# JunkyByte/easy_ViTPose

Measured on NVIDIA H100. Metric: person-crops/sec ViT-B 256x192 bf16, higher is better.
Workload: dtype bf16

## Files before the change

### easy_vitpose_b200/_lib.py

```python
from __future__ import annotations

import ctypes as C
import os

from .build import LIB, build, is_stale

_lib = None


class VpbConfig(C.Structure):
    _fields_ = [("embed_dim", C.c_int32), ("depth", C.c_int32), ("num_heads", C.c_int32),
                ("num_keypoints", C.c_int32), ("max_batch", C.c_int32), ("device", C.c_int32)]


MAX_FRAMES = 64


class VpbFrame(C.Structure):
    _fields_ = [("data", C.c_void_p), ("height", C.c_int32), ("width", C.c_int32), ("pitch_bytes", C.c_int64),
                ("num_boxes", C.c_int32), ("rotation", C.c_int32)]


ROTATIONS = (0, 90, 180, 270)
YUV_MATRICES = {"bt601": 0, "bt709": 1}
# ... 72 lines not shown
    "vpb_infer_frames": (C.c_int, [C.c_void_p, C.POINTER(VpbFrame), C.c_int32, C.c_void_p, C.c_void_p, C.c_void_p, C.c_void_p]),
    "vpb_infer_frames_host": (C.c_int, [C.c_void_p, C.POINTER(VpbFrame), C.c_int32, C.c_void_p, C.c_void_p, C.c_void_p, C.c_void_p]),
    "vpb_submit_frames_host": (C.c_int, [C.c_void_p, C.POINTER(VpbFrame), C.c_int32, C.c_void_p, C.c_void_p, C.c_void_p, C.c_int32]),
    "vpb_preprocess_affine": (C.c_int, [C.POINTER(VpbFrame), C.c_int32, C.c_void_p, C.c_void_p, C.c_void_p]),
    "vpb_infer_affine": (C.c_int, [C.c_void_p, C.POINTER(VpbFrame), C.c_int32, C.c_void_p, C.c_void_p, C.c_void_p, C.c_void_p,
                                   C.c_void_p]),
    "vpb_infer_affine_host": (C.c_int, [C.c_void_p, C.POINTER(VpbFrame), C.c_int32, C.c_void_p, C.c_void_p, C.c_void_p,
                                        C.c_void_p, C.c_void_p]),
    "vpb_create_heads": (C.c_int, [C.POINTER(VpbConfig), C.c_int32, C.c_void_p, C.c_int32, C.POINTER(C.c_void_p)]),
    "vpb_infer_heads": (C.c_int, [C.c_void_p, C.c_void_p, C.c_void_p, C.POINTER(VpbSegment), C.c_int32, C.c_void_p, C.c_void_p,
                                  C.c_void_p, C.c_void_p]),
    "vpb_infer_frames_heads": (C.c_int, [C.c_void_p, C.POINTER(VpbFrame), C.c_int32, C.c_void_p, C.c_void_p, C.c_void_p, C.c_void_p,
                                         C.c_void_p]),
    "vpb_infer_frames_heads_host": (C.c_int, [C.c_void_p, C.POINTER(VpbFrame), C.c_int32, C.c_void_p, C.c_void_p, C.c_void_p,
                                              C.c_void_p, C.c_void_p]),
    "vpb_infer_affine_heads": (C.c_int, [C.c_void_p, C.POINTER(VpbFrame), C.c_int32, C.c_void_p, C.c_void_p, C.c_void_p, C.c_void_p,
                                         C.c_void_p, C.c_void_p]),
    "vpb_infer_affine_heads_host": (C.c_int, [C.c_void_p, C.POINTER(VpbFrame), C.c_int32, C.c_void_p, C.c_void_p, C.c_void_p,
                                              C.c_void_p, C.c_void_p, C.c_void_p]),
    "vpb_infer_frames_yuv": (C.c_int, [C.c_void_p, C.POINTER(VpbFrameYuv), C.c_int32, C.c_int32, C.c_int32, C.c_int32, C.c_void_p,
                                       C.c_void_p, C.c_void_p, C.c_void_p]),
    "vpb_infer_frames_yuv_host": (C.c_int, [C.c_void_p, C.POINTER(VpbFrameYuv), C.c_int32, C.c_int32, C.c_int32, C.c_int32, C.c_void_p,
                                            C.c_void_p, C.c_void_p, C.c_void_p]),
    "vpb_submit_frames_yuv_host": (C.c_int, [C.c_void_p, C.POINTER(VpbFrameYuv), C.c_int32, C.c_int32, C.c_int32, C.c_int32, C.c_void_p,
                                             C.c_void_p, C.c_void_p, C.c_int32]),
    "vpb_infer_affine_yuv": (C.c_int, [C.c_void_p, C.POINTER(VpbFrameYuv), C.c_int32, C.c_int32, C.c_int32, C.c_int32, C.c_void_p,
                                       C.c_void_p, C.c_void_p, C.c_void_p, C.c_void_p]),
    "vpb_infer_affine_yuv_host": (C.c_int, [C.c_void_p, C.POINTER(VpbFrameYuv), C.c_int32, C.c_int32, C.c_int32, C.c_int32, C.c_void_p,
                                            C.c_void_p, C.c_void_p, C.c_void_p, C.c_void_p]),
    "vpb_infer_frames_heads_yuv": (C.c_int, [C.c_void_p, C.POINTER(VpbFrameYuv), C.c_int32, C.c_int32, C.c_int32, C.c_int32, C.c_void_p,
                                             C.c_void_p, C.c_void_p, C.c_void_p, C.c_void_p]),
    "vpb_infer_frames_heads_yuv_host": (C.c_int, [C.c_void_p, C.POINTER(VpbFrameYuv), C.c_int32, C.c_int32, C.c_int32, C.c_int32,
                                                  C.c_void_p, C.c_void_p, C.c_void_p, C.c_void_p, C.c_void_p]),
    "vpb_infer_affine_heads_yuv": (C.c_int, [C.c_void_p, C.POINTER(VpbFrameYuv), C.c_int32, C.c_int32, C.c_int32, C.c_int32, C.c_void_p,
                                             C.c_void_p, C.c_void_p, C.c_void_p, C.c_void_p, C.c_void_p]),
    "vpb_infer_affine_heads_yuv_host": (C.c_int, [C.c_void_p, C.POINTER(VpbFrameYuv), C.c_int32, C.c_int32, C.c_int32, C.c_int32,
                                                  C.c_void_p, C.c_void_p, C.c_void_p, C.c_void_p, C.c_void_p, C.c_void_p]),
    "vpb_host_alloc": (C.c_void_p, [C.c_int64]),
    "vpb_host_free": (None, [C.c_void_p]),
    "vpb_kernel_launches": (C.c_int, [C.c_void_p, C.c_int32]),
    "vpb_cached_graphs": (C.c_int, [C.c_void_p, C.c_int32, C.POINTER(C.c_int32), C.POINTER(C.c_int32)]),
    "vpb_device_bytes": (C.c_int64, [C.c_void_p]),
    "vpb_set_option": (C.c_int, [C.c_void_p, C.c_char_p, C.c_int32]),
    "vpb_set_flip_test": (C.c_int, [C.c_void_p, C.c_void_p, C.c_int32, C.c_int32]),
    "vpb_set_flip_test_heads": (C.c_int, [C.c_void_p, C.c_void_p, C.c_int32, C.c_int32]),
    "vpb_profile_classes": (C.c_int, []),
    "vpb_profile_class_name": (C.c_char_p, [C.c_int32]),
    "vpb_profile_collect": (C.c_int, [C.c_void_p, C.c_void_p, C.c_void_p]),
    "vpb_read_buffer": (C.c_int, [C.c_void_p, C.c_char_p, C.c_void_p, C.c_int64]),
    "vpb_gemm": (C.c_int, [C.c_void_p, C.c_void_p, C.c_void_p, C.c_void_p, C.c_int32, C.c_int32, C.c_int32, C.c_int32,
                           C.c_void_p, C.c_int32, C.c_int32, C.c_int32, C.c_int32, C.c_int32, C.c_void_p]),
    "vpb_debug_gemm": (C.c_int, [C.c_int32, C.c_void_p]),
    "vpb_attention": (C.c_int, [C.c_void_p, C.c_int32, C.c_int32, C.c_int32, C.c_void_p, C.c_void_p]),
    "vpb_debug_attention": (C.c_int, [C.c_int32]),
    "vpb_layernorm": (C.c_int, [C.c_void_p, C.c_void_p, C.c_void_p, C.c_void_p, C.c_int32, C.c_int32, C.c_float, C.c_void_p]),
    "vpb_draw_workspace_bytes": (C.c_int64, [C.c_int32, C.c_int32, C.c_int32]),
    "vpb_draw_poses": (C.c_int, [C.POINTER(VpbCanvas), C.c_int32, C.c_int32, C.c_void_p, C.c_int32, C.c_void_p, C.c_void_p, C.c_int32,
                                 C.c_void_p, C.c_int32, C.c_void_p, C.c_int32, C.c_int32, C.c_float, C.c_void_p, C.c_void_p]),
    "vpb_tracker_create": (C.c_int, [C.c_int32, C.c_int32, C.c_int32, C.c_double, C.c_int32, C.POINTER(C.c_void_p)]),
    "vpb_tracker_destroy": (None, [C.c_void_p]),
    "vpb_tracker_update": (C.c_int, [C.c_void_p, C.c_void_p, C.c_void_p, C.c_void_p, C.c_void_p, C.c_void_p, C.c_void_p]),
    "vpb_tracker_reset": (C.c_int, [C.c_void_p, C.c_int32, C.c_void_p]),
    "vpb_tracker_next_id": (C.c_int, [C.c_void_p, C.POINTER(C.c_int64)]),
    "vpb_tracker_set_next_id": (C.c_int, [C.c_void_p, C.c_int64]),
    "vpb_tracker_status": (C.c_int, [C.c_void_p, C.POINTER(C.c_int32)]),
    "vpb_smoother_create": (C.c_int, [C.c_int32, C.c_int32, C.c_double, C.c_double, C.c_double, C.c_double, C.c_double, C.c_int32,
                                      C.c_int32, C.POINTER(C.c_void_p)]),
    "vpb_smoother_destroy": (None, [C.c_void_p]),
    "vpb_smoother_update": (C.c_int, [C.c_void_p, C.c_void_p, C.c_int32, C.c_void_p, C.c_void_p, C.c_void_p, C.c_void_p, C.c_void_p]),
    "vpb_smoother_reset": (C.c_int, [C.c_void_p, C.c_int32, C.c_void_p]),
    "vpb_smoother_status": (C.c_int, [C.c_void_p, C.POINTER(C.c_int32)]),
    "vpb_oks_nms": (C.c_int, [C.c_void_p, C.c_int32, C.c_int32, C.c_void_p, C.c_int32, C.c_void_p, C.c_void_p, C.c_void_p,
                              C.POINTER(VpbOksNmsParams), C.c_void_p, C.c_void_p, C.c_void_p, C.c_void_p, C.c_void_p]),
    "vpb_oks_iou": (C.c_int, [C.c_void_p, C.c_int32, C.c_int32, C.c_void_p, C.c_int32, C.c_void_p, C.c_void_p, C.c_double,
                              C.c_void_p, C.c_void_p, C.c_void_p]),
    "vpb_coco_eval_workspace_bytes": (C.c_int64, [C.c_int32, C.c_int32]),
    "vpb_coco_eval": (C.c_int, [C.c_int32, C.c_void_p, C.POINTER(VpbCocoGts), C.POINTER(VpbCocoDets), C.c_void_p, C.c_int64, C.c_void_p,
                                C.c_void_p, C.c_void_p, C.c_void_p, C.c_void_p]),
}

EXPORTS_NV12 = {
    "vpb_infer_frames_nv12": (C.c_int, [C.c_void_p, C.POINTER(VpbFrameNv12), C.c_int32, C.c_int32, C.c_void_p, C.c_void_p, C.c_void_p,
                                        C.c_void_p]),
    "vpb_infer_frames_nv12_host": (C.c_int, [C.c_void_p, C.POINTER(VpbFrameNv12), C.c_int32, C.c_int32, C.c_void_p, C.c_void_p,
                                             C.c_void_p, C.c_void_p]),
    "vpb_submit_frames_nv12_host": (C.c_int, [C.c_void_p, C.POINTER(VpbFrameNv12), C.c_int32, C.c_int32, C.c_void_p, C.c_void_p,
                                              C.c_void_p, C.c_int32]),
    "vpb_infer_affine_nv12": (C.c_int, [C.c_void_p, C.POINTER(VpbFrameNv12), C.c_int32, C.c_int32, C.c_void_p, C.c_void_p, C.c_void_p,
                                        C.c_void_p, C.c_void_p]),
    "vpb_infer_affine_nv12_host": (C.c_int, [C.c_void_p, C.POINTER(VpbFrameNv12), C.c_int32, C.c_int32, C.c_void_p, C.c_void_p,
                                             C.c_void_p, C.c_void_p, C.c_void_p]),
}


def lib():
    global _lib
    if _lib is None:
        if not os.path.exists(LIB) or is_stale():
            try:
                build()
            except Exception as exc:
                if not os.path.exists(LIB) or os.environ.get("VPB_ALLOW_STALE", "0") != "1":
                    raise RuntimeError(f"{LIB} is missing or older than its sources and could not be rebuilt ({exc}); build it "
                                       "with `python -m easy_vitpose_b200.build`; there is no fallback implementation") from exc
                import warnings
                warnings.warn(f"loading a STALE {LIB} (VPB_ALLOW_STALE=1): {exc}")
# ... 19 lines not shown
```

### easy_vitpose_b200/csrc/attention.cuh

```cuda
#pragma once
#include <cuda.h>

#include "ptx.cuh"
#include "wgmma.cuh"

namespace vpb {

constexpr int ATT_T = 192;
constexpr int ATT_THREADS = 3 * 128;

template <int HD>
struct AttCfg {
  static_assert(HD == 32 || HD == 64 || HD == 80, "head_dim");
  static constexpr int MAIN = HD == 32 ? 32 : 64;
  static constexpr int TAIL = HD - MAIN;
  static constexpr int MAIN_ROW = MAIN * 2;
  static constexpr int MAIN_BYTES = ATT_T * MAIN_ROW;
  static constexpr int TAIL_BYTES = TAIL ? ATT_T * 32 : 0;
  static constexpr int OPER_BYTES = MAIN_BYTES + TAIL_BYTES;
  static constexpr int STAGE_BYTES = 3 * OPER_BYTES;
  static constexpr int SMEM = 2 * STAGE_BYTES + 1024  + 256 ;
  static_assert(OPER_BYTES % 1024 == 0 && MAIN_BYTES % 1024 == 0, "swizzled boxes keep 1024-byte alignment");
};

struct AttnParams {
  int batch;
  int heads;
  int dim;
  __nv_bfloat16* out;
  long long* dbg;
};

template <int HD, int NPOLY, typename OperandsDone>
__device__ __forceinline__ void attend_item(uint32_t sQ, uint32_t sK, uint32_t sV, __nv_bfloat16* out, int dim, int b, int head, int wg,
                                            int lane, int wq, OperandsDone&& operands_done) {
  using Cfg = AttCfg<HD>;
  static_assert(NPOLY == 0 || NPOLY == 8, "NPOLY");
  constexpr float kLog2e = 1.4426950408889634f;
  float s[ATT_T / 2];
  wgmma_fence();
  {
    const uint64_t qd = wgmma_desc<Cfg::MAIN_ROW>(sQ + wg * 64 * Cfg::MAIN_ROW), kd = wgmma_desc<Cfg::MAIN_ROW>(sK);
#pragma unroll
    for (int k = 0; k < Cfg::MAIN / 16; ++k) wgmma_ss<ATT_T>(s, qd + 2 * k, kd + 2 * k, k != 0);
    if constexpr (Cfg::TAIL > 0)
      wgmma_ss<ATT_T>(s, wgmma_desc<32>(sQ + Cfg::MAIN_BYTES + wg * 64 * 32), wgmma_desc<32>(sK + Cfg::MAIN_BYTES), 1);
  }
  wgmma_commit();
  wgmma_wait<0>();
  wgmma_fence_regs(s);

  float sum[2];
#pragma unroll
  for (int h = 0; h < 2; ++h) {
    float mx = -INFINITY;
#pragma unroll
    for (int j = 0; j < ATT_T / 8; ++j) mx = fmaxf(mx, fmaxf(s[4 * j + 2 * h], s[4 * j + 2 * h + 1]));
    mx = fmaxf(mx, __shfl_xor_sync(0xffffffffu, mx, 1));
    mx = fmaxf(mx, __shfl_xor_sync(0xffffffffu, mx, 2));
    const float mscaled = mx * kLog2e;
    float sm = 0.0f;
#pragma unroll
    for (int j = 0; j < ATT_T / 8; ++j) {
      const float a1 = fmaf(s[4 * j + 2 * h + 1], kLog2e, -mscaled);
      const float e0 = __bfloat162float(__float2bfloat16_rn(ex2_approx(fmaf(s[4 * j + 2 * h], kLog2e, -mscaled))));
      const float e1 = __bfloat162float(__float2bfloat16_rn((NPOLY > 0 && (j & 1) == 0) ? ex2_poly(a1) : ex2_approx(a1)));
      sm += e0 + e1;
      s[4 * j + 2 * h] = e0;
      s[4 * j + 2 * h + 1] = e1;
    }
    sm += __shfl_xor_sync(0xffffffffu, sm, 1);
    sm += __shfl_xor_sync(0xffffffffu, sm, 2);
    sum[h] = sm;
  }

  float o[Cfg::MAIN / 2];
  [[maybe_unused]] float ot[8];
  wgmma_fence();
#pragma unroll
  for (int kk = 0; kk < ATT_T / 16; ++kk) {
    uint32_t a[4];
    a[0] = pack_bf16(s[8 * kk + 0], s[8 * kk + 1]);
    a[1] = pack_bf16(s[8 * kk + 2], s[8 * kk + 3]);
    a[2] = pack_bf16(s[8 * kk + 4], s[8 * kk + 5]);
    a[3] = pack_bf16(s[8 * kk + 6], s[8 * kk + 7]);
    const uint64_t vd = wgmma_desc<Cfg::MAIN_ROW>(sV + kk * 16 * Cfg::MAIN_ROW);
    if constexpr (Cfg::MAIN == 64) wgmma_rs_n64<1>(o, a, vd, kk != 0);
    else wgmma_rs_n32<1>(o, a, vd, kk != 0);
    if constexpr (Cfg::TAIL > 0) wgmma_rs_n16<1>(ot, a, wgmma_desc<32>(sV + Cfg::MAIN_BYTES + kk * 16 * 32), kk != 0);
  }
  wgmma_commit();
  wgmma_wait<0>();
  wgmma_fence_regs(o);
  if constexpr (Cfg::TAIL > 0) wgmma_fence_regs(ot);

  operands_done();

  const int r_lo = wg * 64 + wq * 16 + (lane >> 2);
  const int cq = 2 * (lane & 3);
#pragma unroll
  for (int hh = 0; hh < 2; ++hh) {
    const float inv = 1.0f / sum[hh];
    __nv_bfloat16* orow = out + (static_cast<size_t>(b) * ATT_T + r_lo + 8 * hh) * dim + head * HD;
#pragma unroll
    for (int j = 0; j < Cfg::MAIN / 8; ++j)
      *reinterpret_cast<uint32_t*>(orow + 8 * j + cq) = pack_bf16(o[4 * j + 2 * hh] * inv, o[4 * j + 2 * hh + 1] * inv);
    if constexpr (Cfg::TAIL > 0) {
#pragma unroll
      for (int j = 0; j < 2; ++j)
        *reinterpret_cast<uint32_t*>(orow + Cfg::MAIN + 8 * j + cq) = pack_bf16(ot[4 * j + 2 * hh] * inv, ot[4 * j + 2 * hh + 1] * inv);
    }
  }
}

template <int HD, int NPOLY = 0>
__global__ void __launch_bounds__(ATT_THREADS, 1)
attention_wgmma(const __grid_constant__ CUtensorMap tmap_main, const __grid_constant__ CUtensorMap tmap_tail, const AttnParams p) {
  using Cfg = AttCfg<HD>;
  extern __shared__ uint8_t smem_raw[];
  uint8_t* smem = reinterpret_cast<uint8_t*>((reinterpret_cast<uintptr_t>(smem_raw) + 1023) & ~uintptr_t(1023));
  uint64_t* full = reinterpret_cast<uint64_t*>(smem + 2 * Cfg::STAGE_BYTES);

  const int wg = threadIdx.x >> 7;
  const int tid = threadIdx.x & 127;
  const int lane = threadIdx.x & 31, wq = tid >> 5;
  const int items = p.batch * p.heads;
  const long long t_cta0 = p.dbg ? clock64() : 0;
  long long t_wait = 0;

  if (threadIdx.x == 0) {
    tma_prefetch_desc(&tmap_main);
    if constexpr (Cfg::TAIL > 0) tma_prefetch_desc(&tmap_tail);
    mbar_init(&full[0], 1);
    mbar_init(&full[1], 1);
    fence_mbar_init();
  }
  __syncthreads();
  pdl_launch_dependents();
  pdl_wait();

  auto oper = [&](int q, int o) { return smem + q * Cfg::STAGE_BYTES + o * Cfg::OPER_BYTES; };
  auto load_item = [&](int item, int q) {
    const int b = item / p.heads, h = item % p.heads;
    mbar_expect_tx(&full[q], Cfg::STAGE_BYTES);
#pragma unroll
    for (int o = 0; o < 3; ++o) {
      tma_load_2d(oper(q, o), &tmap_main, &full[q], o * p.dim + h * HD, b * ATT_T);
      if constexpr (Cfg::TAIL > 0) tma_load_2d(oper(q, o) + Cfg::MAIN_BYTES, &tmap_tail, &full[q], o * p.dim + h * HD + Cfg::MAIN, b * ATT_T);
    }
  };
  if (threadIdx.x == 0) {
    if (static_cast<int>(blockIdx.x) < items) load_item(blockIdx.x, 0);
    if (static_cast<int>(blockIdx.x + gridDim.x) < items) load_item(blockIdx.x + gridDim.x, 1);
  }

  int li = 0;
  for (int item = blockIdx.x; item < items; item += gridDim.x, ++li) {
    const int q = li & 1;
    const long long w0 = p.dbg ? clock64() : 0;
    mbar_wait(&full[q], (li >> 1) & 1);
    if (p.dbg && threadIdx.x == 0) t_wait += clock64() - w0;
    const uint32_t sQ = smem_u32(oper(q, 0)), sK = smem_u32(oper(q, 1)), sV = smem_u32(oper(q, 2));

    attend_item<HD, NPOLY>(sQ, sK, sV, p.out, p.dim, item / p.heads, item % p.heads, wg, lane, wq, [&] {
      __syncthreads();
      if (threadIdx.x == 0 && item + 2 * static_cast<int>(gridDim.x) < items) load_item(item + 2 * gridDim.x, q);
    });
  }
  if (p.dbg && threadIdx.x == 0) { p.dbg[blockIdx.x * 8 + 0] = clock64() - t_cta0; p.dbg[blockIdx.x * 8 + 1] = t_wait; p.dbg[blockIdx.x * 8 + 7] = li; }
}

}
```

### easy_vitpose_b200/csrc/engine.cu

```cuda
#include <cuda.h>
#include <cuda_runtime.h>

#include <algorithm>
#include <cmath>
#include <cstdarg>
#include <cstdio>
#include <cstdlib>
#include <cstring>
#include <map>
#include <mutex>
#include <string>
#include <vector>

#include "../../include/vitpose_b200.h"
#include "attention.cuh"
#include "chain.cuh"
#include "decode.cuh"
#include "draw.cuh"
#include "expert_gemm.cuh"
#include "gemm.cuh"
#include "pointwise.cuh"
#include "preprocess.cuh"
#include "oks_nms.cuh"
#include "coco_eval.cuh"
// ... 982 lines not shown
  if (e->use_chain && B >= e->chain_min_batch && !stop && !e->ln_fused && !segs) return backbone_chained(e, B, st);
  auto fuse_ln = [&](GemmParams& p, const float* g, const float* b) {
    if (!ln_fused) return;
    p.ln_gamma = g; p.ln_beta = b; p.ln_out = e->xn; p.ln_counters = e->ln_counters; p.ln_eps = 1e-6f;
  };
  auto standalone_ln = [&](const float* g, const float* b) -> int {
    if (ln_fused) return VPB_OK;
    e->prof.begin(KC_LN, st);
    VPB_TRY(layernorm(e->x, g, b, e->xn, M, D, 1e-6f, st));
    e->prof.end(st);
    return VPB_OK;
  };
  const bool mini = e->ln_in_gemm && !ln_fused && !stop;
  const bool fused = fuse_qkv_attention(e, B);
  const size_t nblk = e->chain_blocks;
  if (mini) CU_TRY(cudaMemsetAsync(e->chain_counters, 0, static_cast<size_t>(e->depth + 1) * 5 * nblk * sizeof(int), st));
  auto ln_gemm = [&](const float* g, const float* b, const LinearW& L, const CUtensorMap& out, int epi, int slot, int kclass) -> int {
    ChainParams p; ChainMaps m;
    memset(&p, 0, sizeof(p));
    p.M = M; p.D = D; p.x = e->x; p.xn = e->xn; p.eps = 1e-6f; p.wave_lag[0] = p.wave_lag[1] = 1 << 20; p.dbg = nullptr;
    p.ln_ctl = e->ln_ctl; p.ln_job_rows = e->ln_job_rows;
    int* ready = e->chain_counters + static_cast<size_t>(slot) * nblk;
    p.ln[0] = {ready, 0, g, b, ready};
    p.num_ln = 1; p.num_phases = 1;
    for (int i = 0; i < CHAIN_MAX_PHASES; ++i) { m.a[i] = e->m_xn; m.w[i] = L.map_c; m.out[i] = out; }
    p.ph[0].N = L.n; p.ph[0].K = L.k; p.ph[0].epi = epi; p.ph[0].bias = L.b; p.ph[0].a_ready = ready; p.ph[0].a_target = 0; p.ph[0].out_done = nullptr;
    e->prof.begin(kclass, st);
    VPB_TRY(chain_launch(e->chain_bn, m, p, st));
    e->prof.end(st);
    return VPB_OK;
  };
  {
    GemmParams p = gp(M, D, 768, e->patch.b, e->x, D);
    fuse_ln(p, e->blocks[0].ln1_g, e->blocks[0].ln1_b);
    e->prof.begin(KC_GEMM_PATCH, st);
    int bn;
    const CUtensorMap* wm;
    VPB_TRY(pick_tile(e->patch, M, &bn, &wm));
    p.rmw = resid_rmw(e->resid_rmw);
    VPB_TRY(gemm_launch(bn, EPI_F32_ADD, e->m_patch_rows, *wm, e->o_x, p, st));
    e->prof.end(st);
  }
  if (stop == 2) return VPB_OK;
  for (int i = 0; i < e->depth; ++i) {
    BlockW& b = e->blocks[i];
    if (mini) {
      VPB_TRY(ln_gemm(b.ln1_g, b.ln1_b, b.qkv, e->o_qkv, EPI_BF16, i * 5 + 4, KC_GEMM_QKV));
    } else {
    VPB_TRY(standalone_ln(b.ln1_g, b.ln1_b));
    if (stop == 3) return VPB_OK;
    e->prof.begin(KC_GEMM_QKV, st);
    if (fused) {
      QkvAttnParams qp;
      qp.batch = B; qp.heads = e->heads; qp.dim = D; qp.bias = b.qkv.b; qp.out = e->attn;
      VPB_TRY(qkv_attention_launch(D / e->heads, e->m_xn_att, b.m_qkv_head, qp, st));
    } else {
      int bn;
      const CUtensorMap* wm;
      VPB_TRY(pick_tile(b.qkv, M, &bn, &wm));
      VPB_TRY(gemm_launch(bn, EPI_BF16, e->m_xn, *wm, e->o_qkv, gp(M, 3 * D, D, b.qkv.b, e->qkv, 3 * D), st));
    }
    e->prof.end(st);
    }
    if (stop == 4) return VPB_OK;
    if (!fused) {
      AttnParams ap;
      ap.batch = B; ap.heads = e->heads; ap.dim = D; ap.out = e->attn; ap.dbg = nullptr;
      e->prof.begin(KC_ATTN, st);
      VPB_TRY(attention_launch(D / e->heads, e->m_qkv_att, e->m_qkv_att_tail, ap, st));
      e->prof.end(st);
    }
    if (stop == 5) return VPB_OK;
    {
      GemmParams p = gp(M, D, D, b.proj.b, e->x, D);
      fuse_ln(p, b.ln2_g, b.ln2_b);
      e->prof.begin(KC_GEMM_PROJ, st);
      int bn;
      const CUtensorMap* wm;
      VPB_TRY(pick_tile(b.proj, M, &bn, &wm));
      p.rmw = resid_rmw(e->resid_rmw);
      VPB_TRY(gemm_launch(bn, EPI_F32_ADD, e->m_attn, *wm, e->o_x, p, st));
      e->prof.end(st);
    }
    if (stop == 6) return VPB_OK;
    if (mini) {
      VPB_TRY(ln_gemm(b.ln2_g, b.ln2_b, b.fc1, e->o_hid, e->gelu_erf ? EPI_BF16_GELU_ERF : EPI_BF16_GELU, (i + 1) * 5 + 1, KC_GEMM_FC1));
    } else {
    VPB_TRY(standalone_ln(b.ln2_g, b.ln2_b));
    e->prof.begin(KC_GEMM_FC1, st);
    {
      int bn;
      const CUtensorMap* wm;
      VPB_TRY(pick_tile(b.fc1, M, &bn, &wm));
      VPB_TRY(gemm_launch(bn, e->gelu_erf ? EPI_BF16_GELU_ERF : EPI_BF16_GELU, e->m_xn, *wm, e->o_hid, gp(M, 4 * D, D, b.fc1.b, e->hid, 4 * D), st));
    }
    e->prof.end(st);
    }
    if (stop == 7) return VPB_OK;
    if (experts) {
      VPB_TRY(fc2_experts(e, b, M, *segs, st));
      if (ln_fused) {
        const bool last = i + 1 == e->depth;
        e->prof.begin(KC_LN, st);
        VPB_TRY(layernorm(e->x, last ? e->lnf_g : e->blocks[i + 1].ln1_g, last ? e->lnf_b : e->blocks[i + 1].ln1_b, e->xn, M, D, 1e-6f, st));
        e->prof.end(st);
      }
    } else {
// ... 1696 lines not shown
extern "C" int vpb_gemm(const void* d_a, const void* d_w, const float* d_bias, void* d_out, int32_t m, int32_t n, int32_t k,
                        int32_t epilogue, const float* d_resid, int32_t resid_mod, int32_t aux0, int32_t aux1, int32_t aux2,
                        int32_t aux3, void* stream) {
  int dev = 0;
  CU_TRY(cudaGetDevice(&dev));
  VPB_TRY(device_check(dev));
  if (!d_a || !d_w || !d_out) return fail(VPB_ERR_ARG, "vpb_gemm: null pointer");
  int bn;
  CUtensorMap ta, tw, tout;
  if (epi_uses_tma(epilogue)) {
    LinearW L;
    L.n = n; L.k = k;
    VPB_TRY(make_tile_maps(L, d_w, n, k));
    const CUtensorMap* wm;
    VPB_TRY(pick_tile(L, m, &bn, &wm));
  } else {
    bn = epilogue == EPI_F32_NCHW ? (n <= 32 ? 32 : 144) : 256;
  }
  if (epilogue == EPI_BF16_RELU_UP && n % bn != 0) return fail(VPB_ERR_ARG, "vpb_gemm: N=%d must be a multiple of %d", n, bn);
  if (epilogue == EPI_F32_NCHW && n != bn) return fail(VPB_ERR_ARG, "vpb_gemm: NCHW epilogue wants W padded to %d rows", bn);
  if (epilogue == EPI_BF16_RELU_UP) {
    const int tile_w = aux3 >> 16, cin = aux3 & 0xffff;
    if ((tile_w * aux2 != 96 && tile_w * aux2 != 128) || cin * 4 != k || aux0 % aux2 != 0 || aux1 % tile_w != 0 || m % (aux0 * aux1) != 0)
      return fail(VPB_ERR_ARG, "vpb_gemm: bad deconv geometry");
    VPB_TRY(make_map_nhwc(&ta, d_a, m / (aux0 * aux1), aux0, aux1, cin, aux2, tile_w));
    VPB_TRY(make_map(&tw, d_w, 4 * n, k, k, bn));
  } else {
    VPB_TRY(make_map(&ta, d_a, m, k, k, 128));
    VPB_TRY(make_map(&tw, d_w, n, k, k, bn));
  }
  VPB_TRY(make_map(&tout, d_w, n, k, k, bn));
  if (epilogue == EPI_BF16 || epilogue == EPI_BF16_GELU || epilogue == EPI_BF16_GELU_ERF) VPB_TRY(make_map(&tout, d_out, m, n, n, 64));
  if (epilogue == EPI_F32_ADD) VPB_TRY(make_map(&tout, d_out, m, n, n, 64, true));
  GemmParams p = gp(m, n, k, d_bias, d_out, n);
  (void)d_resid; (void)resid_mod;
  if (epilogue == EPI_F32_NCHW) { p.n_valid = aux0; p.pix = aux1; }
  if (epilogue == EPI_BF16_RELU_UP) { p.up_h = aux0; p.up_w = aux1; p.up_tr = aux2; p.up_tw = aux3 >> 16; p.up_c = aux3 & 0xffff; }
  return gemm_launch(bn, epilogue, ta, tw, tout, p, static_cast<cudaStream_t>(stream));
}

extern "C" int vpb_attention(const void* d_qkv, int32_t batch, int32_t heads, int32_t head_dim, void* d_out, void* stream) {
  int dev = 0;
  CU_TRY(cudaGetDevice(&dev));
  VPB_TRY(device_check(dev));
  if (!d_qkv || !d_out || batch < 1 || heads < 1) return fail(VPB_ERR_ARG, "vpb_attention: bad argument");
  const int D = heads * head_dim;
  CUtensorMap tm, tt;
  VPB_TRY(make_attn_maps(&tm, &tt, d_qkv, static_cast<uint64_t>(batch) * 192, D, head_dim));
  AttnParams ap;
  ap.batch = batch; ap.heads = heads; ap.dim = D; ap.out = reinterpret_cast<__nv_bfloat16*>(d_out); ap.dbg = g_dbg_buf;
  return attention_launch(head_dim, tm, tt, ap, static_cast<cudaStream_t>(stream));
}

extern "C" int vpb_layernorm(const float* d_x, const float* d_gamma, const float* d_beta, void* d_y, int32_t rows, int32_t dim, float eps,
                             void* stream) {
  if (!d_x || !d_gamma || !d_beta || !d_y) return fail(VPB_ERR_ARG, "vpb_layernorm: null pointer");
  int dev = 0;
  CU_TRY(cudaGetDevice(&dev));
  VPB_TRY(device_check(dev));
  return layernorm(d_x, d_gamma, d_beta, reinterpret_cast<__nv_bfloat16*>(d_y), rows, dim, eps, static_cast<cudaStream_t>(stream));
}
```

### easy_vitpose_b200/csrc/qkv_attention.cuh

```cuda
#pragma once
#include <cuda.h>

#include "attention.cuh"
#include "gemm.cuh"

namespace vpb {

template <int HD>
struct QkvAttCfg {
  using Att = AttCfg<HD>;
  static constexpr int N = 3 * HD;
  static constexpr int A_BYTES = ATT_T * GEMM_BK * 2;
  static constexpr int W_BYTES = HD * GEMM_BK * 2;
  static constexpr int STAGE_BYTES = A_BYTES + 3 * W_BYTES;
  static constexpr int HAND_BYTES = 3 * Att::OPER_BYTES;
  static constexpr int STAGES_RAW = (227 * 1024 - 1024  - 256  - HAND_BYTES) / STAGE_BYTES;
  static constexpr int STAGES = STAGES_RAW > 6 ? 6 : STAGES_RAW;
  static constexpr int SMEM = HAND_BYTES + STAGES * STAGE_BYTES + 1024 + 256;
  static_assert(W_BYTES % 1024 == 0, "W boxes keep the 1024-byte alignment of the swizzle atoms");
  static_assert(STAGES >= 2, "ring too shallow");
};

struct QkvAttnParams {
  int batch;
  int heads;
  int dim;
  const float* bias;
  __nv_bfloat16* out;
};

template <int HD>
__device__ __forceinline__ void qkv_att_produce(int count, uint8_t* ring, uint64_t* full, uint64_t* empty, RingPos& lp, int& ld_item,
                                                int& ld_kb, int items, int num_kb, const QkvAttnParams& p, const CUtensorMap* tmap_x,
                                                const CUtensorMap* tmap_w) {
  using Cfg = QkvAttCfg<HD>;
  for (; count > 0 && ld_item < items; --count) {
    ring_wait_slot(empty, lp);
    uint8_t* st = ring + lp.stage * Cfg::STAGE_BYTES;
    const int b = ld_item / p.heads, h = ld_item % p.heads;
    mbar_expect_tx(&full[lp.stage], Cfg::STAGE_BYTES);
    tma_load_2d(st, tmap_x, &full[lp.stage], ld_kb * GEMM_BK, b * ATT_T);
#pragma unroll
    for (int o = 0; o < 3; ++o) tma_load_2d(st + Cfg::A_BYTES + o * Cfg::W_BYTES, tmap_w, &full[lp.stage], ld_kb * GEMM_BK, o * p.dim + h * HD);
    lp.next(Cfg::STAGES);
    if (++ld_kb == num_kb) { ld_kb = 0; ld_item += gridDim.x; }
  }
}

template <int HD, int NPOLY = 0>
__global__ void __launch_bounds__(ATT_THREADS, 1)
qkv_attention_wgmma(const __grid_constant__ CUtensorMap tmap_x, const __grid_constant__ CUtensorMap tmap_w, const QkvAttnParams p) {
  using Cfg = QkvAttCfg<HD>;
  using Att = AttCfg<HD>;
  constexpr int STAGES = Cfg::STAGES;
  extern __shared__ uint8_t smem_raw[];
  uint8_t* smem = reinterpret_cast<uint8_t*>((reinterpret_cast<uintptr_t>(smem_raw) + 1023) & ~uintptr_t(1023));
  uint8_t* ring = smem + Cfg::HAND_BYTES;
  uint64_t* full = reinterpret_cast<uint64_t*>(ring + STAGES * Cfg::STAGE_BYTES);
  uint64_t* empty = full + STAGES;

  const int wg = threadIdx.x >> 7;
  const int tid = threadIdx.x & 127;
  const int lane = threadIdx.x & 31, wq = tid >> 5;
  const int items = p.batch * p.heads;
  const int num_kb = p.dim / GEMM_BK;

  if (threadIdx.x == 0) {
    tma_prefetch_desc(&tmap_x);
    tma_prefetch_desc(&tmap_w);
    for (int s = 0; s < STAGES; ++s) {
      mbar_init(&full[s], 1);
      mbar_init(&empty[s], ATT_THREADS / 32);
    }
    fence_mbar_init();
  }
  __syncthreads();
  pdl_launch_dependents();
  pdl_wait();

  int ld_item = blockIdx.x, ld_kb = 0;
  RingPos lp;
  auto produce = [&](int count) {
    qkv_att_produce<HD>(count, ring, full, empty, lp, ld_item, ld_kb, items, num_kb, p, &tmap_x, &tmap_w);
  };
  if (threadIdx.x == 0) produce(STAGES);

  const uint32_t sQ = smem_u32(smem), sK = sQ + Att::OPER_BYTES, sV = sQ + 2 * Att::OPER_BYTES;
  RingPos rp;
  for (int item = blockIdx.x; item < items; item += gridDim.x) {
    const int b = item / p.heads, h = item % p.heads;

    float acc[Cfg::N / 2];
#pragma unroll
    for (int i = 0; i < Cfg::N / 2; ++i) acc[i] = 0.0f;
    int prev = -1;
    for (int kb = 0; kb < num_kb; ++kb) {
      mbar_wait(&full[rp.stage], rp.phase);
      const uint32_t sa = smem_u32(ring + rp.stage * Cfg::STAGE_BYTES) + wg * 64 * 128;
      const uint32_t sb = smem_u32(ring + rp.stage * Cfg::STAGE_BYTES + Cfg::A_BYTES);
      const uint64_t ad = wgmma_desc<128>(sa), bd = wgmma_desc<128>(sb);
      wgmma_fence();
#pragma unroll
      for (int k = 0; k < GEMM_BK / 16; ++k) wgmma_ss<Cfg::N>(acc, ad + 2 * k, bd + 2 * k, (kb | k) != 0);
      wgmma_commit();
      wgmma_wait<1>();
      if (prev >= 0) {
        if (lane == 0) mbar_arrive(&empty[prev]);
        if (threadIdx.x == 0) produce(1);
        __syncwarp();
      }
      prev = rp.stage;
      rp.next(STAGES);
    }
    wgmma_wait<0>();
    wgmma_fence_regs(acc);
    if (lane == 0) mbar_arrive(&empty[prev]);

    __syncthreads();
    if (threadIdx.x == 0) produce(1);

    {
      const int r_lo = wg * 64 + wq * 16 + (lane >> 2);
      const int cq = 2 * (lane & 3);
      const uint32_t main_off = r_lo * Att::MAIN_ROW + (lane & 3) * 4;
      const int main_sw = Att::MAIN_ROW == 128 ? (r_lo & 7) : ((r_lo >> 1) & 3);
      const uint32_t tail_off = Att::MAIN_BYTES + r_lo * 32 + (lane & 3) * 4;
      const int tail_sw = (r_lo >> 2) & 1;
#pragma unroll
      for (int j = 0; j < Cfg::N / 8; ++j) {
        const int o = j / (HD / 8), c = (j % (HD / 8)) * 8;
        const float2 b2 = __ldg(reinterpret_cast<const float2*>(p.bias + o * p.dim + h * HD + c + cq));
        const uint32_t lo = pack_bf16(acc[4 * j] + b2.x, acc[4 * j + 1] + b2.y);
        const uint32_t hi = pack_bf16(acc[4 * j + 2] + b2.x, acc[4 * j + 3] + b2.y);
        uint32_t a;
        int row_bytes;
        if (c < Att::MAIN) { a = sQ + o * Att::OPER_BYTES + main_off + (((c >> 3) ^ main_sw) << 4); row_bytes = Att::MAIN_ROW; }
        else { a = sQ + o * Att::OPER_BYTES + tail_off + ((((c - Att::MAIN) >> 3) ^ tail_sw) << 4); row_bytes = 32; }
        sts_u32(a, lo);
        sts_u32(a + 8 * row_bytes, hi);
      }
    }
    fence_proxy_async_smem();
    __syncthreads();

    attend_item<HD, NPOLY>(sQ, sK, sV, p.out, p.dim, b, h, wg, lane, wq, [] {});
  }
}

}
```

### include/vitpose_b200.h

```cpp
#ifndef VITPOSE_B200_H
#define VITPOSE_B200_H

#include <stdint.h>

#ifdef __cplusplus
extern "C" {
#endif

#define VPB_OK 0
#define VPB_ERR_ARG 1
#define VPB_ERR_CUDA 2
#define VPB_ERR_STATE 3

typedef struct vpb_engine vpb_engine;

typedef struct vpb_config {
  int32_t embed_dim;
  int32_t depth;
  int32_t num_heads;
  int32_t num_keypoints;
  int32_t max_batch;
  int32_t device;
} vpb_config;

// ... 200 lines not shown
int vpb_oks_nms(const float* d_kpts, int32_t n_rows, int32_t k, const int32_t* d_counts, int32_t num_frames, const double* d_areas,
                const double* d_scores, const double* h_sigmas, const vpb_oks_nms_params* params, int32_t* d_keep,
                int32_t* d_keep_counts, double* d_scores_out, int32_t* d_status, void* stream);
int vpb_oks_iou(const float* d_kpts, int32_t n_rows, int32_t k, const int32_t* d_counts, int32_t num_frames, const double* d_areas,
                const double* h_sigmas, double vis_thr, float* d_oks, int32_t* d_status, void* stream);

#define VPB_COCO_MAX_GTS 256
#define VPB_COCO_MAX_ROWS 1024
#define VPB_COCO_MAX_K 144
#define VPB_COCO_MAX_IMAGES 1000000
#define VPB_COCO_TOO_MANY_GTS 1
#define VPB_COCO_TOO_MANY_ROWS 2
#define VPB_COCO_BAD_INPUT 4
typedef struct vpb_coco_gts {
  const int32_t* offsets;
  const double* kpts;
  const double* area;
  const double* bbox;
  const int32_t* iscrowd;
  const int32_t* num_keypoints;
  int32_t num_images;
  int32_t num_gts;
} vpb_coco_gts;
typedef struct vpb_coco_dets {
  const double* kpts;
  const double* scores;
  const int32_t* counts;
  const int32_t* frame_image;
  const int32_t* keep;
  const int32_t* keep_counts;
  int32_t n_rows;
  int32_t num_frames;
} vpb_coco_dets;
int64_t vpb_coco_eval_workspace_bytes(int32_t num_images, int32_t num_frames);
int vpb_coco_eval(int32_t k, const double* h_sigmas, const vpb_coco_gts* gts, const vpb_coco_dets* dets, void* d_workspace,
                  int64_t workspace_bytes, double* d_stats, double* d_precision, double* d_recall, int32_t* d_status, void* stream);

int vpb_kernel_launches(const vpb_engine* e, int32_t batch);
int vpb_cached_graphs(const vpb_engine* e, int32_t mixed, int32_t* entries, int32_t* captured);
int64_t vpb_device_bytes(const vpb_engine* e);
int vpb_set_option(vpb_engine* e, const char* name, int32_t value);
int vpb_set_flip_test(vpb_engine* e, const int32_t* h_perm, int32_t k, int32_t shift);
int vpb_set_flip_test_heads(vpb_engine* e, const int32_t* h_perms, int32_t total, int32_t shift);
int vpb_profile_classes(void);
const char* vpb_profile_class_name(int32_t cls);
int vpb_profile_collect(vpb_engine* e, float* ms_per_class, int32_t* launches_per_class);
int vpb_read_buffer(vpb_engine* e, const char* name, void* host_dst, int64_t bytes);

int vpb_gemm(const void* d_a, const void* d_w, const float* d_bias, void* d_out, int32_t m, int32_t n, int32_t k,
             int32_t epilogue, const float* d_resid, int32_t resid_mod, int32_t aux0, int32_t aux1, int32_t aux2,
             int32_t aux3, void* stream);
int vpb_debug_gemm(int32_t stages_limit, void* d_counters);
int vpb_attention(const void* d_qkv, int32_t batch, int32_t heads, int32_t head_dim, void* d_out, void* stream);
int vpb_debug_attention(int32_t flags);
int vpb_layernorm(const float* d_x, const float* d_gamma, const float* d_beta, void* d_y, int32_t rows, int32_t dim,
                  float eps, void* stream);

#ifdef __cplusplus
}
#endif
#endif
```

Before: 11850.

## Split attention QK^T into two key halves to overlap softmax with wgmma

Issues the score wgmma in two halves over the key dimension, so the row max over the first half can be computed while the second half is still in flight. The exp, bf16 packing and P·V wgmma then run per half, letting the first PV wgmma group overlap the exponentials of the second half. The row sum is now taken from the packed bf16 values, and per-phase clock instrumentation plus a debug entry point for the fused QKV-attention kernel are added. The added dbg checks are runtime branches that stay off in production.

Result: faster. 12300 (median of 6 runs) (+3.8%).

```diff
diff --git a/easy_vitpose_b200/_lib.py b/easy_vitpose_b200/_lib.py
--- a/easy_vitpose_b200/_lib.py
+++ b/easy_vitpose_b200/_lib.py
@@ -148,6 +148,7 @@
                            C.c_void_p, C.c_int32, C.c_int32, C.c_int32, C.c_int32, C.c_int32, C.c_void_p]),
     "vpb_debug_gemm": (C.c_int, [C.c_int32, C.c_void_p]),
     "vpb_attention": (C.c_int, [C.c_void_p, C.c_int32, C.c_int32, C.c_int32, C.c_void_p, C.c_void_p]),
+    "vpb_qkv_attention": (C.c_int, [C.c_void_p, C.c_void_p, C.c_void_p, C.c_int32, C.c_int32, C.c_int32, C.c_void_p, C.c_void_p]),
     "vpb_debug_attention": (C.c_int, [C.c_int32]),
     "vpb_layernorm": (C.c_int, [C.c_void_p, C.c_void_p, C.c_void_p, C.c_void_p, C.c_int32, C.c_int32, C.c_float, C.c_void_p]),
     "vpb_draw_workspace_bytes": (C.c_int64, [C.c_int32, C.c_int32, C.c_int32]),
diff --git a/easy_vitpose_b200/csrc/attention.cuh b/easy_vitpose_b200/csrc/attention.cuh
--- a/easy_vitpose_b200/csrc/attention.cuh
+++ b/easy_vitpose_b200/csrc/attention.cuh
@@ -31,70 +31,115 @@
   long long* dbg;
 };
 
+struct PhaseClock {
+  long long* dbg;
+  uint32_t t;
+  __device__ __forceinline__ explicit PhaseClock(long long* d) : dbg(d), t(0) {
+    if (dbg) t = clock_u32();
+  }
+  __device__ __forceinline__ void mark(int slot) {
+    if (dbg) {
+      const uint32_t now = clock_u32();
+      if (threadIdx.x == 0) dbg[slot] += now - t;
+      t = now;
+    }
+  }
+  static __device__ __forceinline__ uint32_t clock_u32() {
+    uint32_t c;
+    asm volatile("mov.u32 %0, %%clock;" : "=r"(c));
+    return c;
+  }
+};
+
 template <int HD, int NPOLY, typename OperandsDone>
 __device__ __forceinline__ void attend_item(uint32_t sQ, uint32_t sK, uint32_t sV, __nv_bfloat16* out, int dim, int b, int head, int wg,
-                                            int lane, int wq, OperandsDone&& operands_done) {
+                                            int lane, int wq, PhaseClock& clk, OperandsDone&& operands_done) {
   using Cfg = AttCfg<HD>;
   static_assert(NPOLY == 0 || NPOLY == 8, "NPOLY");
   constexpr float kLog2e = 1.4426950408889634f;
-  float s[ATT_T / 2];
+  constexpr int KH = ATT_T / 2;
+  float s[2][KH / 2];
   wgmma_fence();
   {
-    const uint64_t qd = wgmma_desc<Cfg::MAIN_ROW>(sQ + wg * 64 * Cfg::MAIN_ROW), kd = wgmma_desc<Cfg::MAIN_ROW>(sK);
-#pragma unroll
-    for (int k = 0; k < Cfg::MAIN / 16; ++k) wgmma_ss<ATT_T>(s, qd + 2 * k, kd + 2 * k, k != 0);
-    if constexpr (Cfg::TAIL > 0)
-      wgmma_ss<ATT_T>(s, wgmma_desc<32>(sQ + Cfg::MAIN_BYTES + wg * 64 * 32), wgmma_desc<32>(sK + Cfg::MAIN_BYTES), 1);
-  }
-  wgmma_commit();
-  wgmma_wait<0>();
-  wgmma_fence_regs(s);
-
-  float sum[2];
+    const uint64_t qd = wgmma_desc<Cfg::MAIN_ROW>(sQ + wg * 64 * Cfg::MAIN_ROW);
+#pragma unroll
+    for (int half = 0; half < 2; ++half) {
+      const uint64_t kd = wgmma_desc<Cfg::MAIN_ROW>(sK + half * KH * Cfg::MAIN_ROW);
+#pragma unroll
+      for (int k = 0; k < Cfg::MAIN / 16; ++k) wgmma_ss<KH>(s[half], qd + 2 * k, kd + 2 * k, k != 0);
+      if constexpr (Cfg::TAIL > 0)
+        wgmma_ss<KH>(s[half], wgmma_desc<32>(sQ + Cfg::MAIN_BYTES + wg * 64 * 32), wgmma_desc<32>(sK + Cfg::MAIN_BYTES + half * KH * 32), 1);
+      wgmma_commit();
+    }
+  }
+
+  float mx[2] = {-INFINITY, -INFINITY};
+  wgmma_wait<1>();
+  wgmma_fence_regs(s[0]);
+#pragma unroll
+  for (int half = 0; half < 2; ++half) {
+    if (half == 1) {
+      wgmma_wait<0>();
+      wgmma_fence_regs(s[1]);
+    }
+#pragma unroll
+    for (int h = 0; h < 2; ++h)
+#pragma unroll
+      for (int j = 0; j < KH / 8; ++j) mx[h] = fmaxf(mx[h], fmaxf(s[half][4 * j + 2 * h], s[half][4 * j + 2 * h + 1]));
+  }
+  clk.mark(3);
+  float mscaled[2];
 #pragma unroll
   for (int h = 0; h < 2; ++h) {
-    float mx = -INFINITY;
-#pragma unroll
-    for (int j = 0; j < ATT_T / 8; ++j) mx = fmaxf(mx, fmaxf(s[4 * j + 2 * h], s[4 * j + 2 * h + 1]));
-    mx = fmaxf(mx, __shfl_xor_sync(0xffffffffu, mx, 1));
-    mx = fmaxf(mx, __shfl_xor_sync(0xffffffffu, mx, 2));
-    const float mscaled = mx * kLog2e;
-    float sm = 0.0f;
-#pragma unroll
-    for (int j = 0; j < ATT_T / 8; ++j) {
-      const float a1 = fmaf(s[4 * j + 2 * h + 1], kLog2e, -mscaled);
-      const float e0 = __bfloat162float(__float2bfloat16_rn(ex2_approx(fmaf(s[4 * j + 2 * h], kLog2e, -mscaled))));
-      const float e1 = __bfloat162float(__float2bfloat16_rn((NPOLY > 0 && (j & 1) == 0) ? ex2_poly(a1) : ex2_approx(a1)));
-      sm += e0 + e1;
-      s[4 * j + 2 * h] = e0;
-      s[4 * j + 2 * h + 1] = e1;
-    }
-    sm += __shfl_xor_sync(0xffffffffu, sm, 1);
-    sm += __shfl_xor_sync(0xffffffffu, sm, 2);
-    sum[h] = sm;
-  }
-
+    mx[h] = fmaxf(mx[h], __shfl_xor_sync(0xffffffffu, mx[h], 1));
+    mx[h] = fmaxf(mx[h], __shfl_xor_sync(0xffffffffu, mx[h], 2));
+    mscaled[h] = mx[h] * kLog2e;
+  }
+
+  float sum[2] = {0.0f, 0.0f};
   float o[Cfg::MAIN / 2];
   [[maybe_unused]] float ot[8];
-  wgmma_fence();
-#pragma unroll
-  for (int kk = 0; kk < ATT_T / 16; ++kk) {
-    uint32_t a[4];
-    a[0] = pack_bf16(s[8 * kk + 0], s[8 * kk + 1]);
-    a[1] = pack_bf16(s[8 * kk + 2], s[8 * kk + 3]);
-    a[2] = pack_bf16(s[8 * kk + 4], s[8 * kk + 5]);
-    a[3] = pack_bf16(s[8 * kk + 6], s[8 * kk + 7]);
-    const uint64_t vd = wgmma_desc<Cfg::MAIN_ROW>(sV + kk * 16 * Cfg::MAIN_ROW);
-    if constexpr (Cfg::MAIN == 64) wgmma_rs_n64<1>(o, a, vd, kk != 0);
-    else wgmma_rs_n32<1>(o, a, vd, kk != 0);
-    if constexpr (Cfg::TAIL > 0) wgmma_rs_n16<1>(ot, a, wgmma_desc<32>(sV + Cfg::MAIN_BYTES + kk * 16 * 32), kk != 0);
-  }
-  wgmma_commit();
+#pragma unroll
+  for (int half = 0; half < 2; ++half) {
+    if (half == 1) wgmma_fence_regs(s[1]);
+    uint32_t pk[KH / 4];
+#pragma unroll
+    for (int h = 0; h < 2; ++h) {
+#pragma unroll
+      for (int jj = 0; jj < KH / 8; ++jj) {
+        const int j = half * (KH / 8) + jj;
+        const float a1 = fmaf(s[half][4 * jj + 2 * h + 1], kLog2e, -mscaled[h]);
+        const float x0 = ex2_approx(fmaf(s[half][4 * jj + 2 * h], kLog2e, -mscaled[h]));
+        const float x1 = (NPOLY > 0 && (j & 1) == 0) ? ex2_poly(a1) : ex2_approx(a1);
+        const uint32_t w = pack_bf16(x0, x1);
+        sum[h] += __uint_as_float(w << 16) + __uint_as_float(w & 0xffff0000u);
+        pk[2 * jj + h] = w;
+      }
+    }
+    wgmma_fence();
+#pragma unroll
+    for (int kh = 0; kh < KH / 16; ++kh) {
+      const int kk = half * (KH / 16) + kh;
+      const uint32_t a[4] = {pk[4 * kh], pk[4 * kh + 1], pk[4 * kh + 2], pk[4 * kh + 3]};
+      const uint64_t vd = wgmma_desc<Cfg::MAIN_ROW>(sV + kk * 16 * Cfg::MAIN_ROW);
+      if constexpr (Cfg::MAIN == 64) wgmma_rs_n64<1>(o, a, vd, kk != 0);
+      else wgmma_rs_n32<1>(o, a, vd, kk != 0);
+      if constexpr (Cfg::TAIL > 0) wgmma_rs_n16<1>(ot, a, wgmma_desc<32>(sV + Cfg::MAIN_BYTES + kk * 16 * 32), kk != 0);
+    }
+    wgmma_commit();
+  }
+  clk.mark(4);
+#pragma unroll
+  for (int h = 0; h < 2; ++h) {
+    sum[h] += __shfl_xor_sync(0xffffffffu, sum[h], 1);
+    sum[h] += __shfl_xor_sync(0xffffffffu, sum[h], 2);
+  }
   wgmma_wait<0>();
   wgmma_fence_regs(o);
   if constexpr (Cfg::TAIL > 0) wgmma_fence_regs(ot);
 
   operands_done();
+  clk.mark(5);
 
   const int r_lo = wg * 64 + wq * 16 + (lane >> 2);
   const int cq = 2 * (lane & 3);
@@ -111,6 +156,7 @@
         *reinterpret_cast<uint32_t*>(orow + Cfg::MAIN + 8 * j + cq) = pack_bf16(ot[4 * j + 2 * hh] * inv, ot[4 * j + 2 * hh + 1] * inv);
     }
   }
+  clk.mark(6);
 }
 
 template <int HD, int NPOLY = 0>
@@ -126,7 +172,7 @@
   const int lane = threadIdx.x & 31, wq = tid >> 5;
   const int items = p.batch * p.heads;
   const long long t_cta0 = p.dbg ? clock64() : 0;
-  long long t_wait = 0;
+  PhaseClock clk(p.dbg ? p.dbg + blockIdx.x * 8 : nullptr);
 
   if (threadIdx.x == 0) {
     tma_prefetch_desc(&tmap_main);
@@ -157,17 +203,17 @@
   int li = 0;
   for (int item = blockIdx.x; item < items; item += gridDim.x, ++li) {
     const int q = li & 1;
-    const long long w0 = p.dbg ? clock64() : 0;
+    clk.mark(2);
     mbar_wait(&full[q], (li >> 1) & 1);
-    if (p.dbg && threadIdx.x == 0) t_wait += clock64() - w0;
+    clk.mark(1);
     const uint32_t sQ = smem_u32(oper(q, 0)), sK = smem_u32(oper(q, 1)), sV = smem_u32(oper(q, 2));
 
-    attend_item<HD, NPOLY>(sQ, sK, sV, p.out, p.dim, item / p.heads, item % p.heads, wg, lane, wq, [&] {
+    attend_item<HD, NPOLY>(sQ, sK, sV, p.out, p.dim, item / p.heads, item % p.heads, wg, lane, wq, clk, [&] {
       __syncthreads();
       if (threadIdx.x == 0 && item + 2 * static_cast<int>(gridDim.x) < items) load_item(item + 2 * gridDim.x, q);
     });
   }
-  if (p.dbg && threadIdx.x == 0) { p.dbg[blockIdx.x * 8 + 0] = clock64() - t_cta0; p.dbg[blockIdx.x * 8 + 1] = t_wait; p.dbg[blockIdx.x * 8 + 7] = li; }
+  if (p.dbg && threadIdx.x == 0) { p.dbg[blockIdx.x * 8 + 0] = clock64() - t_cta0; p.dbg[blockIdx.x * 8 + 7] = li; }
 }
 
 }
diff --git a/easy_vitpose_b200/csrc/engine.cu b/easy_vitpose_b200/csrc/engine.cu
--- a/easy_vitpose_b200/csrc/engine.cu
+++ b/easy_vitpose_b200/csrc/engine.cu
@@ -1058,7 +1058,7 @@
     e->prof.begin(KC_GEMM_QKV, st);
     if (fused) {
       QkvAttnParams qp;
-      qp.batch = B; qp.heads = e->heads; qp.dim = D; qp.bias = b.qkv.b; qp.out = e->attn;
+      qp.batch = B; qp.heads = e->heads; qp.dim = D; qp.bias = b.qkv.b; qp.out = e->attn; qp.dbg = nullptr;
       VPB_TRY(qkv_attention_launch(D / e->heads, e->m_xn_att, b.m_qkv_head, qp, st));
     } else {
       int bn;
@@ -2861,6 +2861,21 @@
   return attention_launch(head_dim, tm, tt, ap, static_cast<cudaStream_t>(stream));
 }
 
+extern "C" int vpb_qkv_attention(const void* d_xn, const void* d_w, const float* d_bias, int32_t batch, int32_t heads, int32_t head_dim,
+                                 void* d_out, void* stream) {
+  int dev = 0;
+  CU_TRY(cudaGetDevice(&dev));
+  VPB_TRY(device_check(dev));
+  const int D = heads * head_dim;
+  if (!d_xn || !d_w || !d_bias || !d_out || batch < 1 || heads < 1 || D % 64 != 0) return fail(VPB_ERR_ARG, "vpb_qkv_attention: bad argument");
+  CUtensorMap tx, tw;
+  VPB_TRY(make_map(&tx, d_xn, static_cast<uint64_t>(batch) * 192, D, D, 192));
+  VPB_TRY(make_map(&tw, d_w, 3 * static_cast<uint64_t>(D), D, D, head_dim));
+  QkvAttnParams qp;
+  qp.batch = batch; qp.heads = heads; qp.dim = D; qp.bias = d_bias; qp.out = reinterpret_cast<__nv_bfloat16*>(d_out); qp.dbg = g_dbg_buf;
+  return qkv_attention_launch(head_dim, tx, tw, qp, static_cast<cudaStream_t>(stream));
+}
+
 extern "C" int vpb_layernorm(const float* d_x, const float* d_gamma, const float* d_beta, void* d_y, int32_t rows, int32_t dim, float eps,
                              void* stream) {
   if (!d_x || !d_gamma || !d_beta || !d_y) return fail(VPB_ERR_ARG, "vpb_layernorm: null pointer");
diff --git a/easy_vitpose_b200/csrc/qkv_attention.cuh b/easy_vitpose_b200/csrc/qkv_attention.cuh
--- a/easy_vitpose_b200/csrc/qkv_attention.cuh
+++ b/easy_vitpose_b200/csrc/qkv_attention.cuh
@@ -27,6 +27,7 @@
   int dim;
   const float* bias;
   __nv_bfloat16* out;
+  long long* dbg;
 };
 
 template <int HD>
@@ -64,6 +65,7 @@
   const int lane = threadIdx.x & 31, wq = tid >> 5;
   const int items = p.batch * p.heads;
   const int num_kb = p.dim / GEMM_BK;
+  PhaseClock clk(p.dbg ? p.dbg + blockIdx.x * 8 : nullptr);
 
   if (threadIdx.x == 0) {
     tma_prefetch_desc(&tmap_x);
@@ -95,7 +97,9 @@
     for (int i = 0; i < Cfg::N / 2; ++i) acc[i] = 0.0f;
     int prev = -1;
     for (int kb = 0; kb < num_kb; ++kb) {
+      const long long w0 = p.dbg ? clock64() : 0;
       mbar_wait(&full[rp.stage], rp.phase);
+      if (p.dbg && threadIdx.x == 0) p.dbg[blockIdx.x * 8 + 1] += clock64() - w0;
       const uint32_t sa = smem_u32(ring + rp.stage * Cfg::STAGE_BYTES) + wg * 64 * 128;
       const uint32_t sb = smem_u32(ring + rp.stage * Cfg::STAGE_BYTES + Cfg::A_BYTES);
       const uint64_t ad = wgmma_desc<128>(sa), bd = wgmma_desc<128>(sb);
@@ -115,6 +119,7 @@
     wgmma_wait<0>();
     wgmma_fence_regs(acc);
     if (lane == 0) mbar_arrive(&empty[prev]);
+    clk.mark(0);
 
     __syncthreads();
     if (threadIdx.x == 0) produce(1);
@@ -142,9 +147,11 @@
     }
     fence_proxy_async_smem();
     __syncthreads();
+    clk.mark(2);
 
-    attend_item<HD, NPOLY>(sQ, sK, sV, p.out, p.dim, b, h, wg, lane, wq, [] {});
+    attend_item<HD, NPOLY>(sQ, sK, sV, p.out, p.dim, b, h, wg, lane, wq, clk, [] {});
   }
+  if (p.dbg && threadIdx.x == 0) p.dbg[blockIdx.x * 8 + 7] = (items - 1 - blockIdx.x) / gridDim.x + 1;
 }
 
 }
diff --git a/include/vitpose_b200.h b/include/vitpose_b200.h
--- a/include/vitpose_b200.h
+++ b/include/vitpose_b200.h
@@ -276,6 +276,8 @@
              int32_t aux3, void* stream);
 int vpb_debug_gemm(int32_t stages_limit, void* d_counters);
 int vpb_attention(const void* d_qkv, int32_t batch, int32_t heads, int32_t head_dim, void* d_out, void* stream);
+int vpb_qkv_attention(const void* d_xn, const void* d_w, const float* d_bias, int32_t batch, int32_t heads, int32_t head_dim,
+                      void* d_out, void* stream);
 int vpb_debug_attention(int32_t flags);
 int vpb_layernorm(const float* d_x, const float* d_gamma, const float* d_beta, void* d_y, int32_t rows, int32_t dim,
                   float eps, void* stream);
```
